# ChenWu98/cycle-diffusion

Hardware: AMD Instinct MI355X
Metric: images/sec, SD-v1.4 512px CycleDiffusion 100+100 steps, 1/2/4/8 MI355X (higher is better)
Workload: dtype fp16; 1 GPU; C2: Stable-Diffusion-v1.4-shaped U-Net + KL-f8 VAE, 512x512, custom_steps=99 white_box_steps=100 eta=0.1 skip 0, 1 trial, encoder scale 1, decoder CFG 3; batch_per_gpu=4, global_batch=4, parallelism=dp1, steps_per_launch_set=5, launch_set_cap=16, launch_sets_in_flight_per_gpu=1, images_in_flight_per_gpu=20, distributed=single process, weights=synthetic(seed=0)

## Files before the change

### cycle-diffusion_amd/csrc/attn.hip

```cpp
#include "common.h"
#include "kernels.h"

namespace cd {

namespace {

constexpr int KT = 64;

template <int DQK, int DV, int DH, int NBUF, bool VTOK, int KG, int NWV = 4>
__global__ __launch_bounds__(64 * NWV, DV <= 96 ? (KG == 32 ? (DV <= 64 ? 4 : 3) : 2) : 1) void k_attention(AttnParams p) {
  constexpr int NT = 64 * NWV;
  constexpr int KLD = DQK + 8;
  constexpr int VLD = KT + 8;
  constexpr int NKS = DQK / 16;
  constexpr int NDT = DV / 32;
  constexpr int CPR = DQK / 8;
  constexpr int NKR = (KT * CPR + NT - 1) / NT;
  constexpr bool ONES = DH > 0;
  constexpr int VS = DV <= 32 ? 32 : (DV <= 96 ? 96 : 160);
  constexpr int CPRV = ONES ? DH / 8 + 1 : DV / 8;
  constexpr int NVR = VTOK ? (KT * CPRV + NT - 1) / NT : (DV * 8 + NT - 1) / NT;
  constexpr int VBUF = VTOK ? KT * VS : DV * VLD;
  static_assert(!ONES || (DH < DV && (DH & 7) == 0 && ((DH >> 2) & 1) == 0), "ones row placement");
  __shared__ __attribute__((aligned(16))) bf16_t Ks[NBUF][KT * KLD];
  __shared__ __attribute__((aligned(16))) bf16_t Vs[NBUF][VBUF];

  const int tid = threadIdx.x, lane = tid & 63, wave = tid >> 6;
  const int qi = lane & 31, half = lane >> 5;
  const int h = blockIdx.y, b = blockIdx.z;
  const int q0 = blockIdx.x * (32 * NWV) + wave * 32;
  const int D = ONES ? DH : p.D;

  const bf16_t* qb = p.q + (int64_t)b * p.q_bs + h * D;
  const bf16_t* kb = p.k + (int64_t)b * p.k_bs + h * D;
  const bf16_t* vtb = VTOK ? p.v + (int64_t)b * p.v_bs + h * D
                           : p.vt + ((int64_t)b * p.H + h) * (int64_t)p.vt_dpad * p.vt_tpad;

  bf16x8 qf[NKS];
  const float qsc = p.scale * 1.44269504088896340736f;
  {
    const int q = q0 + qi;
#pragma unroll
    for (int ks = 0; ks < NKS; ++ks) {
      const int d0 = ks * 16 + 8 * half;
      uint4 raw = make_uint4(0, 0, 0, 0);
      if (q < p.Tq && d0 < D) raw = *(const uint4*)(qb + (int64_t)q * p.ldq + d0);
      if (!p.q_log2) {
        float f[8];
        unpack8(raw, f);
#pragma unroll
        for (int e = 0; e < 8; ++e) f[e] *= qsc;
        raw = pack8(f);
      }
      qf[ks] = *(bf16x8*)&raw;
    }
  }

  constexpr unsigned kNoLoad = 0x80000000u;
  const unsigned k_bytes = p.Tk > 0 ? (unsigned)(((int64_t)(p.Tk - 1) * p.ldk + D) * 2) : 0u;
  const unsigned v_bytes = VTOK ? (p.Tk > 0 ? (unsigned)(((int64_t)(p.Tk - 1) * p.ldv + D) * 2) : 0u)
                                : (unsigned)((int64_t)p.vt_dpad * p.vt_tpad * 2);
  const __amdgpu_buffer_rsrc_t rs_k = __builtin_amdgcn_make_buffer_rsrc((void*)kb, 0, k_bytes, 0x00020000);
  const __amdgpu_buffer_rsrc_t rs_v = __builtin_amdgcn_make_buffer_rsrc((void*)vtb, 0, v_bytes, 0x00020000);
  unsigned k_voff[NKR], v_voff[NVR];
  int k_loff[NKR], v_loff[NVR];
  bool v_ones[NVR];
#pragma unroll
  for (int i = 0; i < NKR; ++i) {
    const int id = tid + i * NT;
    const int row = id / CPR, ch = id % CPR;
    const bool ok = id < KT * CPR && ch * 8 < D;
    k_voff[i] = ok ? (unsigned)((row * p.ldk + ch * 8) * 2) : kNoLoad;
    k_loff[i] = id < KT * CPR ? row * KLD + ch * 8 : -1;
  }
#pragma unroll
  for (int i = 0; i < NVR; ++i) {
    const int id = tid + i * NT;
    if (VTOK) {
      const int row = id / CPRV, ch = id % CPRV;
      const bool data = id < KT * CPRV && ch * 8 < D;
      v_voff[i] = data ? (unsigned)((row * p.ldv + ch * 8) * 2) : kNoLoad;
      v_loff[i] = id < KT * CPRV ? row * VS + ch * 8 : -1;
      v_ones[i] = ONES && ch * 8 == DH;
    } else {
      const int row = id >> 3, ch = id & 7;
      v_voff[i] = row < DV ? (unsigned)((row * p.vt_tpad + ch * 8) * 2) : kNoLoad;
      v_loff[i] = row < DV ? row * VLD + (ch >> 1) * 16 + (ch & 1) * 4 : -1;
      v_ones[i] = ONES && row == DH;
    }
  }
  uint4 kreg[NKR], vreg[NVR];
  auto fetch = [&](int key0) {
    const unsigned k_toff = (unsigned)(key0 * p.ldk * 2);
    const unsigned v_toff = (unsigned)(VTOK ? key0 * p.ldv * 2 : key0 * 2);
#pragma unroll
    for (int i = 0; i < NKR; ++i)
      kreg[i] = __builtin_bit_cast(uint4, __builtin_amdgcn_raw_buffer_load_b128(rs_k, k_voff[i] + k_toff, 0, 0));
#pragma unroll
    for (int i = 0; i < NVR; ++i)
      vreg[i] = __builtin_bit_cast(uint4, __builtin_amdgcn_raw_buffer_load_b128(rs_v, v_voff[i] + v_toff, 0, 0));
  };
  auto commit = [&](int buf) {
#pragma unroll
    for (int i = 0; i < NKR; ++i)
      if (k_loff[i] >= 0) *(uint4*)(&Ks[buf][k_loff[i]]) = kreg[i];
#pragma unroll
    for (int i = 0; i < NVR; ++i) {
      uint4 v = vreg[i];
      if (VTOK) {
        if (v_ones[i]) v = make_uint4(kOnePair & 0xffffu, 0, 0, 0);
        if (v_loff[i] >= 0) *(uint4*)(&Vs[buf][v_loff[i]]) = v;
      } else {
        if (v_ones[i]) v = make_uint4(kOnePair, kOnePair, kOnePair, kOnePair);
        if (v_loff[i] >= 0) {
          *(uint2*)(&Vs[buf][v_loff[i]]) = make_uint2(v.x, v.y);
          *(uint2*)(&Vs[buf][v_loff[i] + 8]) = make_uint2(v.z, v.w);
        }
      }
    }
  };
  const int vtr_off = ((4 * half + ((lane & 15) >> 2)) * VS + 16 * ((lane >> 4) & 1) + 4 * (lane & 3));

  f32x16 o[NDT];
#pragma unroll
  for (int i = 0; i < NDT; ++i)
#pragma unroll
    for (int r = 0; r < 16; ++r) o[i][r] = 0.f;
  f32x16 negm;
#pragma unroll
  for (int r = 0; r < 16; ++r) negm[r] = 0.f;
  float l_part = 0.f;
  constexpr float kDefer = 8.0f;

  const int ntiles = (p.Tk + KT - 1) / KT;
  fetch(0);
  commit(0);
  __syncthreads();
  for (int t = 0; t < ntiles; ++t) {
    const int key0 = t * KT;
    const int buf = NBUF == 2 ? (t & 1) : 0;
    const bool more = t + 1 < ntiles;
    if (more) fetch(key0 + KT);
    const bf16_t* Kt = Ks[buf];
    const bf16_t* Vt = Vs[buf];

#pragma unroll
    for (int g = 0; g < KT / KG; ++g) {
      constexpr int HPG = KG / 32;
      f32x16 s[HPG];
      {
        bf16x8 kf[HPG][NKS];
#pragma unroll
        for (int kh = 0; kh < HPG; ++kh)
#pragma unroll
          for (int ks = 0; ks < NKS; ++ks)
            kf[kh][ks] = *(const bf16x8*)(Kt + ((g * HPG + kh) * 32 + qi) * KLD + ks * 16 + 8 * half);
        if (KG == 64) __builtin_amdgcn_sched_barrier(0);
#pragma unroll
        for (int ks = 0; ks < NKS; ++ks)
#pragma unroll
          for (int kh = 0; kh < HPG; ++kh)
            s[kh] = CD_MFMA_32x32x16(kf[kh][ks], qf[ks], ks == 0 ? negm : s[kh]);
      }
      if (key0 + KT > p.Tk || p.causal) {
        const int kmax = p.causal ? min(p.Tk - 1, q0 + qi) : p.Tk - 1;
#pragma unroll
        for (int kh = 0; kh < HPG; ++kh)
#pragma unroll
          for (int r = 0; r < 16; ++r) {
            const int key = key0 + (g * HPG + kh) * 32 + (r & 3) + 8 * (r >> 2) + 4 * half;
            s[kh][r] = key <= kmax ? s[kh][r] : -INFINITY;
          }
      }
      float mx = __builtin_amdgcn_fmed3f(s[HPG - 1][14], s[HPG - 1][15], INFINITY);
      if (HPG == 2) {
#pragma unroll
        for (int r = 0; r < 14; r += 2)
          asm("v_max3_f32 %0, %1, %2, %3" : "=v"(mx) : "v"(mx), "v"(s[1][r]), "v"(s[1][r + 1]));
      }
#pragma unroll
      for (int r = 0; r < (HPG == 2 ? 16 : 14); r += 2)
        asm("v_max3_f32 %0, %1, %2, %3" : "=v"(mx) : "v"(mx), "v"(s[0][r]), "v"(s[0][r + 1]));
      const bool first = t == 0 && g == 0;
      if (first || __any(mx > kDefer)) {
        const float mxq = fmaxf(mx, __shfl_xor(mx, 32));
        float delta = first ? mxq : fmaxf(mxq, 0.f);
        delta = delta == -INFINITY ? 0.f : delta;
        const float alpha = first ? 1.f : __builtin_amdgcn_exp2f(-delta);
#pragma unroll
        for (int kh = 0; kh < HPG; ++kh)
#pragma unroll
          for (int r = 0; r < 16; ++r) s[kh][r] -= delta;
#pragma unroll
        for (int r = 0; r < 16; ++r) negm[r] -= delta;
#pragma unroll
        for (int i = 0; i < NDT; ++i)
#pragma unroll
          for (int r = 0; r < 16; ++r) o[i][r] *= alpha;
        l_part *= alpha;
      }
      uint32_t pw[HPG][8];
      float ps = 0.f;
#pragma unroll
      for (int kh = 0; kh < HPG; ++kh)
#pragma unroll
        for (int r = 0; r < 16; r += 2) {
          const float e0 = __builtin_amdgcn_exp2f(s[kh][r]);
          const float e1 = __builtin_amdgcn_exp2f(s[kh][r + 1]);
          if (!ONES) ps += e0 + e1;
          pw[kh][r >> 1] = pack2_prob(e0, e1);
        }
      if (!ONES) l_part += ps;

#pragma unroll
      for (int kh = 0; kh < HPG; ++kh)
#pragma unroll
        for (int s2 = 0; s2 < 2; ++s2) {
          const uint4 praw = make_uint4(pw[kh][4 * s2], pw[kh][4 * s2 + 1], pw[kh][4 * s2 + 2], pw[kh][4 * s2 + 3]);
          const bf16x8 pf = __builtin_bit_cast(bf16x8, praw);
          const int k16 = (g * HPG + kh) * 32 + 16 * s2;
#pragma unroll
          for (int dt = 0; dt < NDT; ++dt) {
            bf16x8 vf;
            if (VTOK) {
              typedef __attribute__((address_space(3))) bf16x4* lds4_t;
              const bf16_t* vr = Vt + vtr_off + k16 * VS + dt * 32;
              const bf16x4 lo = __builtin_amdgcn_ds_read_tr16_b64_v4i16((lds4_t)vr);
              const bf16x4 hi = __builtin_amdgcn_ds_read_tr16_b64_v4i16((lds4_t)(vr + 8 * VS));
              vf = __builtin_shufflevector(lo, hi, 0, 1, 2, 3, 4, 5, 6, 7);
            } else {
              vf = *(const bf16x8*)(Vt + (dt * 32 + qi) * VLD + k16 + 8 * half);
            }
            o[dt] = CD_MFMA_32x32x16(vf, pf, o[dt]);
          }
        }
    }

    if (NBUF == 1) __syncthreads();
    if (more) commit(NBUF == 2 ? (buf ^ 1) : 0);
    __syncthreads();
  }

  float l_tot;
  if (ONES) {
    constexpr int L = DH % 32;
    const float lv = o[DH / 32][(L & 3) + 4 * (L >> 3)];
    l_tot = __shfl(lv, qi);
  } else {
    l_tot = l_part + __shfl_xor(l_part, 32);
  }
  const float inv = 1.0f / l_tot;
  const int q = q0 + qi;
  if (q < p.Tq) {
    bf16_t* ob = p.o + (int64_t)b * p.o_bs + (int64_t)q * p.ldo + h * D;
#pragma unroll
    for (int dt = 0; dt < NDT; ++dt)
#pragma unroll
      for (int rq = 0; rq < 4; ++rq) {
        const int d0 = dt * 32 + 8 * rq + 4 * half;
        if (d0 < D) {
          float bb[4] = {0.f, 0.f, 0.f, 0.f};
          if (p.obias) {
#pragma unroll
            for (int e = 0; e < 4; ++e) bb[e] = p.obias[h * D + d0 + e];
          }
          uint2 pk;
          pk.x = pack2(o[dt][rq * 4 + 0] * inv + bb[0], o[dt][rq * 4 + 1] * inv + bb[1]);
          pk.y = pack2(o[dt][rq * 4 + 2] * inv + bb[2], o[dt][rq * 4 + 3] * inv + bb[3]);
          *(uint2*)(ob + d0) = pk;
        }
      }
  }
}

template <int NWV>
__global__ __launch_bounds__(64 * NWV, 4) void k_attention_d40(AttnParams p) {
#if defined(__HIP_DEVICE_COMPILE__)
  static_assert(NWV == 8, "one K copy per wave and tile");
  typedef __attribute__((address_space(3))) void* lptr_t;
  constexpr int D = 40, NKS = 3, ROWB = 128;
  constexpr int KBUF = KT * ROWB;
  constexpr int VBUF = 48 * ROWB;
  constexpr int BUF = KBUF + VBUF;
  __shared__ __attribute__((aligned(1024))) char lds[2 * BUF];

  const int tid = threadIdx.x, lane = tid & 63;
  const int wave = __builtin_amdgcn_readfirstlane(tid >> 6);
  const int qi = lane & 31, half = lane >> 5;
  const int h = blockIdx.y, b = blockIdx.z;
  const int q0 = blockIdx.x * (32 * NWV) + wave * 32;

  const bf16_t* qb = p.q + (int64_t)b * p.q_bs + h * D;
  const bf16_t* kb = p.k + (int64_t)b * p.k_bs + h * D;
  const bf16_t* vtb = p.vt + ((int64_t)b * p.H + h) * (int64_t)p.vt_dpad * p.vt_tpad;

  bf16x8 qf[NKS];
  {
    const float qsc = p.scale * 1.44269504088896340736f;
    const int q = q0 + qi;
#pragma unroll
    for (int ks = 0; ks < NKS; ++ks) {
      const int d0 = ks * 16 + 8 * half;
      uint4 raw = make_uint4(0, 0, 0, 0);
      if (q < p.Tq && d0 < D) raw = *(const uint4*)(qb + (int64_t)q * p.ldq + d0);
      if (!p.q_log2) {
        float f[8];
        unpack8(raw, f);
#pragma unroll
        for (int e = 0; e < 8; ++e) f[e] *= qsc;
        raw = pack8(f);
      }
      qf[ks] = *(bf16x8*)&raw;
    }
  }

  constexpr unsigned kNoLoad = 0x80000000u;
  const unsigned k_bytes = p.Tk > 0 ? (unsigned)(((int64_t)(p.Tk - 1) * p.ldk + D) * 2) : 0u;
  const unsigned v_bytes = (unsigned)((int64_t)p.vt_dpad * p.vt_tpad * 2);
  const __amdgpu_buffer_rsrc_t rs_k = __builtin_amdgcn_make_buffer_rsrc((void*)kb, 0, k_bytes, 0x00020000);
  const __amdgpu_buffer_rsrc_t rs_v = __builtin_amdgcn_make_buffer_rsrc((void*)vtb, 0, v_bytes, 0x00020000);
  unsigned k_voff, v_voff;
  {
    const int row = 8 * wave + (lane >> 3);
    const int lc = (lane & 7) ^ ((row >> 1) & 7);
    const int pc = (row >> 2) & 3;
    const int key = (row & ~12) | ((((pc & 1) << 1) | (pc >> 1)) << 2);
    k_voff = lc < D / 8 ? (unsigned)((key * p.ldk + lc * 8) * 2) : kNoLoad;
    v_voff = (row < D && row < p.vt_dpad) ? (unsigned)((row * p.vt_tpad + lc * 8) * 2) : kNoLoad;
  }
  auto fetch = [&](int key0, int buf) {
    char* kd = lds + buf * BUF + wave * 1024;
    __builtin_amdgcn_raw_ptr_buffer_load_lds(rs_k, (lptr_t)kd, 16, k_voff + (unsigned)(key0 * p.ldk * 2), 0, 0, 0);
    if (wave < D / 8)
      __builtin_amdgcn_raw_ptr_buffer_load_lds(rs_v, (lptr_t)(kd + KBUF), 16, v_voff + (unsigned)(key0 * 2), 0, 0, 0);
  };
  if (wave == 5 || wave == 6) {
    const uint4 v = lane < 8 ? make_uint4(kOnePair, kOnePair, kOnePair, kOnePair) : make_uint4(0, 0, 0, 0);
    *(uint4*)(lds + (wave - 5) * BUF + KBUF + D * ROWB + lane * 16) = v;
  }

  const int sw = (qi >> 1) & 7;
  const int kf_off = qi * ROWB;
  const int vf_off = KBUF + qi * ROWB;
  const int tm = lane & 15, tg = lane >> 4;
  const int vt_off = KBUF + (32 + tm) * ROWB;
  const int vt_sw = ((32 + tm) >> 1) & 7, vt_lc = ((tg & 1) << 1) | (tg >> 1);

  f32x16 o0;
  f32x4 ot0 = {0.f, 0.f, 0.f, 0.f}, ot1 = {0.f, 0.f, 0.f, 0.f};
  f32x16 negm;
#pragma unroll
  for (int r = 0; r < 16; ++r) { o0[r] = 0.f; negm[r] = 0.f; }
  constexpr float kDefer = 8.0f;

  const int ntiles = (p.Tk + KT - 1) / KT;
  fetch(0, 0);
  asm volatile("s_waitcnt vmcnt(0)" ::: "memory");
  __syncthreads();
  for (int t = 0; t < ntiles; ++t) {
    const int key0 = t * KT;
    const int buf = t & 1;
    if (t + 1 < ntiles) fetch(key0 + KT, buf ^ 1);
    const char* Bt = lds + buf * BUF;
#pragma unroll
    for (int g = 0; g < 2; ++g) {
      f32x16 s;
      {
        bf16x8 kf[NKS];
#pragma unroll
        for (int ks = 0; ks < NKS; ++ks)
          kf[ks] = *(const bf16x8*)(Bt + kf_off + g * 32 * ROWB + (((2 * ks + half) ^ sw) << 4));
#pragma unroll
        for (int ks = 0; ks < NKS; ++ks) s = CD_MFMA_32x32x16(kf[ks], qf[ks], ks == 0 ? negm : s);
      }
      if (key0 + KT > p.Tk || p.causal) {
        const int kmax = p.causal ? min(p.Tk - 1, q0 + qi) : p.Tk - 1;
#pragma unroll
        for (int r = 0; r < 16; ++r) {
          const int row = (r & 3) + 8 * (r >> 2) + 4 * half;
          const int pc = (row >> 2) & 3;
          const int key = key0 + g * 32 + ((row & ~12) | ((((pc & 1) << 1) | (pc >> 1)) << 2));
          s[r] = key <= kmax ? s[r] : -INFINITY;
        }
      }
      float mx = __builtin_amdgcn_fmed3f(s[14], s[15], INFINITY);
#pragma unroll
      for (int r = 0; r < 14; r += 2) asm("v_max3_f32 %0, %1, %2, %3" : "=v"(mx) : "v"(mx), "v"(s[r]), "v"(s[r + 1]));
      const bool first = t == 0 && g == 0;
      if (first || __any(mx > kDefer)) {
        const float mxq = fmaxf(mx, __shfl_xor(mx, 32));
        float delta = first ? mxq : fmaxf(mxq, 0.f);
        delta = delta == -INFINITY ? 0.f : delta;
        const float alpha = first ? 1.f : __builtin_amdgcn_exp2f(-delta);
#pragma unroll
        for (int r = 0; r < 16; ++r) { s[r] -= delta; negm[r] -= delta; o0[r] *= alpha; }
        const float a0 = __shfl(alpha, lane & 15), a1 = __shfl(alpha, 16 + (lane & 15));
#pragma unroll
        for (int r = 0; r < 4; ++r) { ot0[r] *= a0; ot1[r] *= a1; }
      }
      uint32_t pw[8];
#pragma unroll
      for (int r = 0; r < 16; r += 2)
        pw[r >> 1] = pack2_prob(__builtin_amdgcn_exp2f(s[r]), __builtin_amdgcn_exp2f(s[r + 1]));
#pragma unroll
      for (int s2 = 0; s2 < 2; ++s2) {
        const bf16x8 vf = *(const bf16x8*)(Bt + vf_off + (((4 * g + 2 * s2 + half) ^ sw) << 4));
        const uint4 praw = make_uint4(pw[4 * s2], pw[4 * s2 + 1], pw[4 * s2 + 2], pw[4 * s2 + 3]);
        o0 = CD_MFMA_32x32x16(vf, __builtin_bit_cast(bf16x8, praw), o0);
      }
      {
        uint32_t xa[4], ya[4];
#pragma unroll
        for (int i = 0; i < 4; ++i) {
          const auto r2 = __builtin_amdgcn_permlane16_swap(pw[i], pw[4 + i], false, false);
          xa[i] = r2[0]; ya[i] = r2[1];
        }
        const bf16x8 va = *(const bf16x8*)(Bt + vt_off + (((4 * g + vt_lc) ^ vt_sw) << 4));
        ot0 = CD_MFMA_16x16x32(va, __builtin_bit_cast(bf16x8, make_uint4(xa[0], xa[1], xa[2], xa[3])), ot0);
        ot1 = CD_MFMA_16x16x32(va, __builtin_bit_cast(bf16x8, make_uint4(ya[0], ya[1], ya[2], ya[3])), ot1);
      }
    }
    asm volatile("s_waitcnt vmcnt(0)" ::: "memory");
    __syncthreads();
  }

  const float l0 = __shfl(ot0[0], 32 + (lane & 15)), l1 = __shfl(ot1[0], 32 + (lane & 15));
  {
    const int q = q0 + qi;
    const float inv = 1.0f / ((qi & 16) ? l1 : l0);
    if (q < p.Tq) {
      bf16_t* ob = p.o + (int64_t)b * p.o_bs + (int64_t)q * p.ldo + h * D;
#pragma unroll
      for (int rq = 0; rq < 4; ++rq) {
        const int d0 = 8 * rq + 4 * half;
        float bb[4] = {0.f, 0.f, 0.f, 0.f};
        if (p.obias) {
#pragma unroll
          for (int e = 0; e < 4; ++e) bb[e] = p.obias[h * D + d0 + e];
        }
        uint2 pk;
        pk.x = pack2(o0[rq * 4 + 0] * inv + bb[0], o0[rq * 4 + 1] * inv + bb[1]);
        pk.y = pack2(o0[rq * 4 + 2] * inv + bb[2], o0[rq * 4 + 3] * inv + bb[3]);
        *(uint2*)(ob + d0) = pk;
      }
    }
  }
  if (tg < 2) {
    const int d0 = 32 + 4 * tg;
    float bb[4] = {0.f, 0.f, 0.f, 0.f};
    if (p.obias) {
#pragma unroll
      for (int e = 0; e < 4; ++e) bb[e] = p.obias[h * D + d0 + e];
    }
#pragma unroll
    for (int qh = 0; qh < 2; ++qh) {
      const int q = q0 + tm + 16 * qh;
      const f32x4 ov = qh ? ot1 : ot0;
      const float inv = 1.0f / (qh ? l1 : l0);
      if (q < p.Tq) {
        uint2 pk;
        pk.x = pack2(ov[0] * inv + bb[0], ov[1] * inv + bb[1]);
        pk.y = pack2(ov[2] * inv + bb[2], ov[3] * inv + bb[3]);
        *(uint2*)(p.o + (int64_t)b * p.o_bs + (int64_t)q * p.ldo + h * D + d0) = pk;
      }
    }
  }
#endif
}

__global__ __launch_bounds__(256) void k_transpose_v(const bf16_t* __restrict__ v, int ldv, int64_t v_bs,
                                                     bf16_t* __restrict__ vt, int H, int Tk, int D,
                                                     int Dpad, int Tpad) {
  extern __shared__ __attribute__((aligned(16))) bf16_t tile[];
  const int key0 = blockIdx.x * 64, h = blockIdx.y, b = blockIdx.z;
  const int ldt = D + 2;
  const int cpr = D / 8;
  for (int id = threadIdx.x; id < 64 * cpr; id += 256) {
    const int row = id / cpr, ch = id % cpr;
    uint4 raw = make_uint4(0, 0, 0, 0);
    if (key0 + row < Tk) raw = *(const uint4*)(v + (int64_t)b * v_bs + (int64_t)(key0 + row) * ldv + h * D + ch * 8);
    bf16_t* d = tile + row * ldt + ch * 8;
    const bf16_t* rs = (const bf16_t*)&raw;
#pragma unroll
    for (int e = 0; e < 8; ++e) d[e] = rs[e];
  }
  __syncthreads();
  bf16_t* ob = vt + ((int64_t)b * H + h) * (int64_t)Dpad * Tpad;
  for (int id = threadIdx.x; id < Dpad * 64; id += 256) {
    const int d = id >> 6, key = id & 63;
    bf16_t val = 0;
    if (d < D) val = tile[key * ldt + d];
    ob[(int64_t)d * Tpad + key0 + key] = val;
  }
}

template <int DQK, int DV>
__global__ __launch_bounds__(256, DV <= 96 ? 2 : 1) void k_cross_attention_ctrl(CtrlAttnParams p) {
  constexpr int NT = 256, CK = kCtrlKeys, NG = CK / 32;
  constexpr int KLD = DQK + 8, NKS = DQK / 16, NDT = DV / 32, CPR = DQK / 8;
  constexpr int VS = DV <= 32 ? 32 : (DV <= 96 ? 96 : 160), CPV = VS / 8;
  __shared__ __attribute__((aligned(16))) bf16_t Ks[2][CK * KLD];
  __shared__ __attribute__((aligned(16))) bf16_t Vs[2][CK * VS];

  const int tid = threadIdx.x, lane = tid & 63, wave = tid >> 6;
  const int qi = lane & 31, half = lane >> 5;
  const int h = blockIdx.y, b = blockIdx.z, bs = b % p.B_src;
  const int q0 = blockIdx.x * 128 + wave * 32;
  const int D = p.D, L = p.L;

#pragma unroll
  for (int src = 0; src < 2; ++src) {
    const bf16_t* kb = (src == 0 ? p.k_src + (int64_t)bs * p.k_bs : p.k_own + (int64_t)b * p.k_bs) + h * D;
    const bf16_t* vb = (src == 0 ? p.va : p.vb) + (int64_t)b * p.v_bs + h * D;
    for (int id = tid; id < CK * CPR; id += NT) {
      const int row = id / CPR, ch = id % CPR;
      uint4 raw = make_uint4(0, 0, 0, 0);
      if (row < L && ch * 8 < D) raw = *(const uint4*)(kb + (int64_t)row * p.ldk + ch * 8);
      *(uint4*)(&Ks[src][row * KLD + ch * 8]) = raw;
    }
    for (int id = tid; id < CK * CPV; id += NT) {
      const int row = id / CPV, ch = id % CPV;
      uint4 raw = make_uint4(0, 0, 0, 0);
      if (row < L && ch * 8 < D) raw = *(const uint4*)(vb + (int64_t)row * p.ldv + ch * 8);
      *(uint4*)(&Vs[src][row * VS + ch * 8]) = raw;
    }
  }
  __syncthreads();

  const int vtr_off = ((4 * half + ((lane & 15) >> 2)) * VS + 16 * ((lane >> 4) & 1) + 4 * (lane & 3));
  const float qsc = p.scale * 1.44269504088896340736f;
  f32x16 o[NDT];
#pragma unroll
  for (int i = 0; i < NDT; ++i)
#pragma unroll
    for (int r = 0; r < 16; ++r) o[i][r] = 0.f;

#pragma unroll
  for (int src = 0; src < 2; ++src) {
    const bf16_t* qb = (src == 0 ? p.q_src + (int64_t)bs * p.q_bs : p.q_own + (int64_t)b * p.q_bs) + h * D;
    bf16x8 qf[NKS];
    {
      const int q = q0 + qi;
#pragma unroll
      for (int ks = 0; ks < NKS; ++ks) {
        const int d0 = ks * 16 + 8 * half;
        uint4 raw = make_uint4(0, 0, 0, 0);
        if (q < p.Tq && d0 < D) raw = *(const uint4*)(qb + (int64_t)q * p.ldq + d0);
        if (!p.q_log2) {
          float f[8];
          unpack8(raw, f);
#pragma unroll
          for (int e = 0; e < 8; ++e) f[e] *= qsc;
          raw = pack8(f);
        }
        qf[ks] = *(bf16x8*)&raw;
      }
    }
    const bf16_t* Kt = Ks[src];
    const bf16_t* Vt = Vs[src];
    f32x16 s[NG];
#pragma unroll
    for (int g = 0; g < NG; ++g) {
#pragma unroll
      for (int r = 0; r < 16; ++r) s[g][r] = 0.f;
#pragma unroll
      for (int ks = 0; ks < NKS; ++ks) {
        const bf16x8 kf = *(const bf16x8*)(Kt + (g * 32 + qi) * KLD + ks * 16 + 8 * half);
        s[g] = CD_MFMA_32x32x16(kf, qf[ks], s[g]);
      }
    }
    float mx = -INFINITY;
#pragma unroll
    for (int g = 0; g < NG; ++g)
#pragma unroll
      for (int r = 0; r < 16; ++r) {
        const int key = g * 32 + (r & 3) + 8 * (r >> 2) + 4 * half;
        s[g][r] = key < L ? s[g][r] : -INFINITY;
        mx = fmaxf(mx, s[g][r]);
      }
    mx = fmaxf(mx, __shfl_xor(mx, 32));
    float ps = 0.f;
#pragma unroll
    for (int g = 0; g < NG; ++g)
#pragma unroll
      for (int r = 0; r < 16; ++r) {
        s[g][r] = __builtin_amdgcn_exp2f(s[g][r] - mx);
        ps += s[g][r];
      }
    ps += __shfl_xor(ps, 32);
    const float inv = 256.0f / ps;
#pragma unroll
    for (int g = 0; g < NG; ++g) {
      uint32_t pw[8];
#pragma unroll
      for (int r = 0; r < 16; r += 2) pw[r >> 1] = pack2_prob(s[g][r] * inv, s[g][r + 1] * inv);
#pragma unroll
      for (int s2 = 0; s2 < 2; ++s2) {
        const uint4 praw = make_uint4(pw[4 * s2], pw[4 * s2 + 1], pw[4 * s2 + 2], pw[4 * s2 + 3]);
        const bf16x8 pf = __builtin_bit_cast(bf16x8, praw);
        const int k16 = g * 32 + 16 * s2;
#pragma unroll
        for (int dt = 0; dt < NDT; ++dt) {
          typedef __attribute__((address_space(3))) bf16x4* lds4_t;
          const bf16_t* vr = Vt + vtr_off + k16 * VS + dt * 32;
          const bf16x4 lo = __builtin_amdgcn_ds_read_tr16_b64_v4i16((lds4_t)vr);
          const bf16x4 hi = __builtin_amdgcn_ds_read_tr16_b64_v4i16((lds4_t)(vr + 8 * VS));
          const bf16x8 vf = __builtin_shufflevector(lo, hi, 0, 1, 2, 3, 4, 5, 6, 7);
          o[dt] = CD_MFMA_32x32x16(vf, pf, o[dt]);
        }
      }
    }
  }

  const int q = q0 + qi;
  if (q < p.Tq) {
    constexpr float kUnscale = 1.0f / 256.0f;
    bf16_t* ob = p.o + (int64_t)b * p.o_bs + (int64_t)q * p.ldo + h * D;
#pragma unroll
    for (int dt = 0; dt < NDT; ++dt)
#pragma unroll
      for (int rq = 0; rq < 4; ++rq) {
        const int d0 = dt * 32 + 8 * rq + 4 * half;
        if (d0 < D) {
          uint2 pk;
          pk.x = pack2(o[dt][rq * 4 + 0] * kUnscale, o[dt][rq * 4 + 1] * kUnscale);
          pk.y = pack2(o[dt][rq * 4 + 2] * kUnscale, o[dt][rq * 4 + 3] * kUnscale);
          *(uint2*)(ob + d0) = pk;
        }
      }
  }
}

__global__ __launch_bounds__(256) void k_ctrl_values(const bf16_t* __restrict__ v, const float* __restrict__ M,
                                                     const float* __restrict__ alpha, const float* __restrict__ w, int B_ctrl,
                                                     int L, int C, bf16_t* __restrict__ va, bf16_t* __restrict__ vb) {
  const int i = blockIdx.x, r = blockIdx.y, s = r % B_ctrl;
  const float* Mi = M + ((int64_t)s * L + i) * L;
  const float* al = alpha + (int64_t)s * L;
  const float* ww = w + (int64_t)s * L;
  const bf16_t* vr = v + (int64_t)r * L * C;
  const float bi = (1.0f - al[i]) * ww[i];
  for (int c = threadIdx.x; c < C; c += 256) {
    float acc = 0.f;
    for (int j = 0; j < L; ++j) {
      const float m = Mi[j] * al[j] * ww[j];
      if (m != 0.f) acc = fmaf(m, bf2f(vr[(int64_t)j * C + c]), acc);
    }
    va[((int64_t)r * L + i) * C + c] = f2bf(acc);
    vb[((int64_t)r * L + i) * C + c] = f2bf(bi * bf2f(vr[(int64_t)i * C + c]));
  }
}

}

void launch_cross_attention_ctrl(hipStream_t st, const CtrlAttnParams& p) {
  CD_CHECK(p.B > 0 && p.B_src > 0 && p.H > 0 && p.Tq > 0, "cross-attention control: empty launch");
  CD_CHECK(p.L > 0 && p.L <= kCtrlKeys, "cross-attention control: context length %d above the %d keys the kernel keeps resident",
           p.L, kCtrlKeys);
  CD_CHECK((p.ldq % 8) == 0 && (p.ldk % 8) == 0 && (p.ldv % 8) == 0 && (p.ldo % 4) == 0 && (p.q_bs % 8) == 0 &&
               (p.k_bs % 8) == 0 && (p.v_bs % 8) == 0 && (p.o_bs % 4) == 0,
           "cross-attention control: leading dims");
  CD_CHECK((((uintptr_t)p.q_own | (uintptr_t)p.q_src | (uintptr_t)p.k_own | (uintptr_t)p.k_src | (uintptr_t)p.va |
             (uintptr_t)p.vb) & 15) == 0 && ((uintptr_t)p.o & 7) == 0, "cross-attention control: pointer alignment");
  const dim3 grid(ceil_div(p.Tq, 128), p.H, p.B);
#define CD_CTRL(DQK, DV) hipLaunchKernelGGL((k_cross_attention_ctrl<DQK, DV>), grid, dim3(256), 0, st, p)
  switch (p.D) {
    case 32: CD_CTRL(32, 32); break;
    case 40: CD_CTRL(48, 64); break;
    case 64: CD_CTRL(64, 64); break;
    case 80: CD_CTRL(80, 96); break;
    case 160: CD_CTRL(160, 160); break;
    default: CD_CHECK(false, "cross-attention control: head dim %d unsupported (32, 40, 64, 80, 160)", p.D);
  }
#undef CD_CTRL
}

void launch_ctrl_values(hipStream_t st, const bf16_t* v, const float* M, const float* alpha, const float* w, int rows,
                        int B_ctrl, int L, int C, bf16_t* va, bf16_t* vb) {
  CD_CHECK(rows > 0 && B_ctrl > 0 && L > 0 && C > 0, "control values: empty launch");
  hipLaunchKernelGGL(k_ctrl_values, dim3(L, rows), dim3(256), 0, st, v, M, alpha, w, B_ctrl, L, C, va, vb);
}

void launch_attention(hipStream_t st, const AttnParams& p) {
  CD_CHECK(p.D % 8 == 0 && p.D <= 160, "attention: head dim %d unsupported by the fused kernel", p.D);
  CD_CHECK((p.v != nullptr) != (p.vt != nullptr), "attention: exactly one of v (token-major) / vt (transposed)");
  if (p.vt) CD_CHECK(p.vt_tpad % KT == 0 && p.vt_tpad >= round_up(p.Tk, KT), "attention: V^T key padding");
  else CD_CHECK((p.ldv % 8) == 0 && ((uintptr_t)p.v & 15) == 0, "attention: V row stride / alignment");
  CD_CHECK((p.ldq % 8) == 0 && (p.ldk % 8) == 0 && (p.ldo % 4) == 0, "attention: leading dims");
  dim3 grid(ceil_div(p.Tq, 128), p.H, p.B);
#define CD_LAUNCH_KG(DQK, DV, DH, NBUF, KG)                                                                  \
  do {                                                                                                      \
    if (p.v) hipLaunchKernelGGL((k_attention<DQK, DV, DH, NBUF, true, KG>), grid, dim3(256), 0, st, p);      \
    else hipLaunchKernelGGL((k_attention<DQK, DV, DH, NBUF, false, KG>), grid, dim3(256), 0, st, p);         \
  } while (0)
#define CD_ATTN(DQK, DV, DH, NBUF) CD_LAUNCH_KG(DQK, DV, DH, NBUF, 64)
  if (p.D == 40 && p.Tq >= 1024 && p.Tk >= 1024 && p.vt) {
    const bool aligned16 = ((((uintptr_t)p.q | (uintptr_t)p.k | (uintptr_t)p.vt | (uintptr_t)p.o) & 15) == 0) &&
                           (p.ldq % 8) == 0 && (p.ldk % 8) == 0 && (p.ldo % 8) == 0 && (p.q_bs % 8) == 0 && (p.k_bs % 8) == 0 &&
                           (p.o_bs % 8) == 0;
    if (p.vt_dpad >= 40 && aligned16 && (p.vt_tpad % 8) == 0 && p.vt_tpad >= ceil_div(p.Tk, 64) * 64 &&
        (int64_t)p.Tk * p.ldk * 2 < (1ll << 31) && (int64_t)p.vt_dpad * p.vt_tpad * 2 < (1ll << 31))
      hipLaunchKernelGGL((k_attention_d40<8>), dim3(ceil_div(p.Tq, 256), p.H, p.B), dim3(512), 0, st, p);
    else
      hipLaunchKernelGGL((k_attention<48, 64, 40, 2, false, 32, 8>), dim3(ceil_div(p.Tq, 256), p.H, p.B), dim3(512), 0, st,
                         p);
  } else if (p.D == 40) CD_LAUNCH_KG(48, 64, 40, 2, 32);
  else if (p.D == 80) CD_LAUNCH_KG(80, 96, 80, 2, 32);
  else if (p.D <= 32) CD_ATTN(32, 32, 0, 2);
  else if (p.D <= 48) CD_ATTN(48, 64, 0, 2);
  else if (p.D <= 64) CD_ATTN(64, 64, 0, 2);
  else if (p.D <= 80) CD_ATTN(80, 96, 0, 2);
  else if (p.D <= 96) CD_ATTN(96, 96, 0, 2);
  else if (p.D <= 128) CD_ATTN(128, 128, 0, 1);
  else CD_ATTN(160, 160, 0, 1);
#undef CD_ATTN
#undef CD_LAUNCH_KG
}

void launch_transpose_v(hipStream_t st, const bf16_t* v, int ldv, int64_t v_bs, bf16_t* vt, int B,
                        int H, int Tk, int D, int Dpad, int Tpad) {
  CD_CHECK(D % 8 == 0 && Tpad % 64 == 0, "transpose_v: D %% 8, Tpad %% 64");
  const size_t lds = (size_t)64 * (D + 2) * sizeof(bf16_t);
  hipLaunchKernelGGL(k_transpose_v, dim3(Tpad / 64, H, B), dim3(256), lds, st, v, ldv, v_bs, vt, H,
                     Tk, D, Dpad, Tpad);
}

}
```

Baseline: 3.549 images/s.

## Add slab-based cross-attention kernel keeping all short-context K/V resident in LDS

Adds a specialised cross-attention kernel for short key sequences (≤96 tokens, e.g. the 77 text tokens) with head dims 40/80/160. Each block loads a 320-channel slab of K and V for all keys into LDS once, then loops over query chunks with several heads per block, using a single-pass softmax (no online rescaling), transposed LDS reads for V, and buffer loads/stores. The grid is sized from the device CU count so work spreads across the GPU. It can be disabled with an environment variable. The trade-offs are extra specialised code, higher LDS use per block, and a fixed max-minus-8 exponent shift in the softmax.

```diff
diff --git a/cycle-diffusion_amd/csrc/attn.hip b/cycle-diffusion_amd/csrc/attn.hip
--- a/cycle-diffusion_amd/csrc/attn.hip
+++ b/cycle-diffusion_amd/csrc/attn.hip
@@ -629,6 +629,224 @@
         }
       }
   }
+}
+
+constexpr int kSlabC = 320;
+constexpr int kSlabKeys = 96;
+typedef __attribute__((ext_vector_type(2))) float f32x2;
+
+__device__ inline float prob_pair_sum(uint32_t pw, float acc) {
+#if CD_ACT_FP16
+  typedef __attribute__((ext_vector_type(2))) _Float16 h2;
+  const h2 one = {(_Float16)1.0f, (_Float16)1.0f};
+  return __builtin_amdgcn_fdot2(__builtin_bit_cast(h2, pw), one, acc, false);
+#else
+  return acc + __uint_as_float(pw << 16) + __uint_as_float(pw & 0xffff0000u);
+#endif
+}
+
+template <int D, int GR>
+__global__ __launch_bounds__(512, 1) void k_cross_attention_slab(AttnParams p, int qchunk) {
+#if defined(__HIP_DEVICE_COMPILE__)
+  constexpr int NW = 8, NT = 64 * NW, SC = kSlabC, NG = GR + 1, CK = NG * 32;
+  constexpr int HPS = SC / D;
+  constexpr int QB = 32 * NW / HPS;
+  constexpr int NKS = (D + 15) / 16, NDT = (D + 31) / 32;
+  constexpr int KROW = SC * 2;
+  constexpr int VS = SC + 32;
+  constexpr int CPR = SC / 8;
+  constexpr int NR = (CK * CPR + NT - 1) / NT;
+  static_assert(SC % D == 0 && NW % HPS == 0 && D % 8 == 0 && CK <= kSlabKeys, "slab geometry");
+  __shared__ __attribute__((aligned(1024))) char Ks[CK * KROW];
+  __shared__ __attribute__((aligned(16))) bf16_t Vs[CK * VS];
+
+  const int tid = threadIdx.x, lane = tid & 63;
+  const int wave = __builtin_amdgcn_readfirstlane(tid >> 6);
+  const int qi = lane & 31, half = lane >> 5;
+  const int slab = blockIdx.y, b = blockIdx.z;
+  const int Tk = p.Tk;
+
+  {
+    constexpr unsigned kNoLoad = 0x80000000u;
+    const bf16_t* kb = p.k + (int64_t)b * p.k_bs + slab * SC;
+    const bf16_t* vb = p.v + (int64_t)b * p.v_bs + slab * SC;
+    const unsigned k_bytes = (unsigned)(((int64_t)(Tk - 1) * p.ldk + SC) * 2);
+    const unsigned v_bytes = (unsigned)(((int64_t)(Tk - 1) * p.ldv + SC) * 2);
+    const __amdgpu_buffer_rsrc_t rs_k = __builtin_amdgcn_make_buffer_rsrc((void*)kb, 0, k_bytes, 0x00020000);
+    const __amdgpu_buffer_rsrc_t rs_v = __builtin_amdgcn_make_buffer_rsrc((void*)vb, 0, v_bytes, 0x00020000);
+    uint4 kr[NR], vr[NR];
+#pragma unroll
+    for (int i = 0; i < NR; ++i) {
+      const int id = tid + i * NT;
+      const int row = id / CPR, ch = id % CPR;
+      const bool ok = id < CK * CPR;
+      kr[i] = __builtin_bit_cast(uint4, __builtin_amdgcn_raw_buffer_load_b128(
+                                            rs_k, ok ? (unsigned)((row * p.ldk + ch * 8) * 2) : kNoLoad, 0, 0));
+      vr[i] = __builtin_bit_cast(uint4, __builtin_amdgcn_raw_buffer_load_b128(
+                                            rs_v, ok ? (unsigned)((row * p.ldv + ch * 8) * 2) : kNoLoad, 0, 0));
+    }
+#pragma unroll
+    for (int i = 0; i < NR; ++i) {
+      const int id = tid + i * NT;
+      const int row = id / CPR, ch = id % CPR;
+      if (id < CK * CPR) {
+        *(uint4*)(Ks + row * KROW + (((ch & ~7) | ((ch & 7) ^ ((row >> 1) & 7))) << 4)) = kr[i];
+        *(uint4*)(&Vs[row * VS + ch * 8]) = vr[i];
+      }
+    }
+  }
+  __syncthreads();
+
+  const int hoff = (wave % HPS) * D;
+  const int sub = wave / HPS;
+  const int qbeg = blockIdx.x * qchunk, qend = min(p.Tq, qbeg + qchunk);
+  const float qsc = p.scale * 1.44269504088896340736f;
+  constexpr unsigned kNoLane = 0x80000000u;
+  const __amdgpu_buffer_rsrc_t rs_q = __builtin_amdgcn_make_buffer_rsrc(
+      (void*)(p.q + (int64_t)b * p.q_bs + slab * SC), 0, (unsigned)(((int64_t)(p.Tq - 1) * p.ldq + SC) * 2), 0x00020000);
+  const __amdgpu_buffer_rsrc_t rs_o = __builtin_amdgcn_make_buffer_rsrc(
+      (void*)(p.o + (int64_t)b * p.o_bs + slab * SC), 0, (unsigned)(((int64_t)(p.Tq - 1) * p.ldo + SC) * 2), 0x00020000);
+
+  auto load_q = [&](int q0, uint4* raw) {
+    const int q = q0 + sub * 32 + qi;
+#pragma unroll
+    for (int ks = 0; ks < NKS; ++ks) {
+      const int d0 = ks * 16 + 8 * half;
+      const unsigned off = (q < qend && d0 < D) ? (unsigned)((q * p.ldq + hoff + d0) * 2) : kNoLane;
+      raw[ks] = __builtin_bit_cast(uint4, __builtin_amdgcn_raw_buffer_load_b128(rs_q, off, 0, 0));
+    }
+  };
+
+  const int ksw = (qi >> 1) & 7;
+  int kf_off[NKS];
+  bool kf_zero[NKS];
+#pragma unroll
+  for (int ks = 0; ks < NKS; ++ks) {
+    kf_zero[ks] = ks * 16 + 8 * half >= D;
+    const int c = hoff / 8 + 2 * ks + half - (kf_zero[ks] ? 1 : 0);
+    kf_off[ks] = qi * KROW + (((c & ~7) | ((c & 7) ^ ksw)) << 4);
+  }
+  const int vtr_off = (4 * half + ((lane & 15) >> 2)) * VS + 16 * ((lane >> 4) & 1) + 4 * (lane & 3) + hoff;
+
+  auto read_k = [&](int g, int ks) {
+    bf16x8 kf = *(const bf16x8*)(Ks + g * 32 * KROW + kf_off[ks]);
+    if (NKS * 16 > D && ks == NKS - 1 && kf_zero[ks]) kf = bf16x8{0, 0, 0, 0, 0, 0, 0, 0};
+    return kf;
+  };
+  auto read_v = [&](int g, int s2, int dt) {
+    typedef __attribute__((address_space(3))) bf16x4* lds4_t;
+    const bf16_t* vr = Vs + vtr_off + (g * 32 + 16 * s2) * VS + dt * 32;
+    const bf16x4 lo = __builtin_amdgcn_ds_read_tr16_b64_v4i16((lds4_t)vr);
+    const bf16x4 hi = __builtin_amdgcn_ds_read_tr16_b64_v4i16((lds4_t)(vr + 8 * VS));
+    return (bf16x8)__builtin_shufflevector(lo, hi, 0, 1, 2, 3, 4, 5, 6, 7);
+  };
+  f32x16 kmask, kzero;
+#pragma unroll
+  for (int r = 0; r < 16; ++r) {
+    kmask[r] = GR * 32 + (r & 3) + 8 * (r >> 2) + 4 * half < Tk ? 0.f : -INFINITY;
+    kzero[r] = 0.f;
+  }
+
+  uint4 qraw[NKS];
+  load_q(qbeg, qraw);
+  typedef decltype(__builtin_amdgcn_raw_buffer_load_b128(rs_o, 0, 0, 0)) b128_t;
+#pragma unroll
+  for (int i = 0; i < (D + 15) / 16; ++i)
+    __builtin_amdgcn_raw_buffer_store_b128(__builtin_bit_cast(b128_t, make_uint4(0, 0, 0, 0)), rs_o, kNoLane + 16u * i, 0,
+                                           0);
+  for (int q0 = qbeg; q0 < qend; q0 += QB) {
+    bf16x8 qf[NKS];
+#pragma unroll
+    for (int ks = 0; ks < NKS; ++ks) {
+      uint4 raw = qraw[ks];
+      if (!p.q_log2) {
+        float f[8];
+        unpack8(raw, f);
+#pragma unroll
+        for (int e = 0; e < 8; ++e) f[e] *= qsc;
+        raw = pack8(f);
+      }
+      qf[ks] = __builtin_bit_cast(bf16x8, raw);
+    }
+    load_q(q0 + QB, qraw);
+
+    f32x16 s[NG];
+#pragma unroll
+    for (int g = 0; g < NG; ++g) {
+      bf16x8 kf[NKS];
+#pragma unroll
+      for (int ks = 0; ks < NKS; ++ks) kf[ks] = read_k(g, ks);
+      __builtin_amdgcn_sched_barrier(0);
+#pragma unroll
+      for (int ks = 0; ks < NKS; ++ks) s[g] = CD_MFMA_32x32x16(kf[ks], qf[ks], ks == 0 ? (g == GR ? kmask : kzero) : s[g]);
+    }
+    float mg[NG];
+#pragma unroll
+    for (int g = 0; g < NG; ++g) {
+      mg[g] = __builtin_amdgcn_fmed3f(s[g][14], s[g][15], INFINITY);
+#pragma unroll
+      for (int r = 0; r < 14; r += 2)
+        asm("v_max3_f32 %0, %1, %2, %3" : "=v"(mg[g]) : "v"(mg[g]), "v"(s[g][r]), "v"(s[g][r + 1]));
+    }
+    float mx = mg[0];
+#pragma unroll
+    for (int g = 1; g < NG; ++g) mx = fmaxf(mx, mg[g]);
+    mx = fmaxf(mx, __shfl_xor(mx, 32));
+    const f32x2 mm = {mx - 8.0f, mx - 8.0f};
+    uint32_t pw[NG][8];
+    float ps = 0.f;
+#pragma unroll
+    for (int g = 0; g < NG; ++g)
+#pragma unroll
+      for (int r = 0; r < 16; r += 2) {
+        const f32x2 t = f32x2{s[g][r], s[g][r + 1]} - mm;
+        pw[g][r >> 1] = pack2_prob(__builtin_amdgcn_exp2f(t.x), __builtin_amdgcn_exp2f(t.y));
+        ps = prob_pair_sum(pw[g][r >> 1], ps);
+      }
+    ps += __shfl_xor(ps, 32);
+    const float inv1 = 1.0f / ps;
+    const f32x2 inv = {inv1, inv1};
+
+    f32x16 o[NDT];
+#pragma unroll
+    for (int i = 0; i < NDT; ++i)
+#pragma unroll
+      for (int r = 0; r < 16; ++r) o[i][r] = 0.f;
+#pragma unroll
+    for (int g = 0; g < NG; ++g)
+#pragma unroll
+      for (int s2 = 0; s2 < 2; ++s2) {
+        const uint4 praw = make_uint4(pw[g][4 * s2], pw[g][4 * s2 + 1], pw[g][4 * s2 + 2], pw[g][4 * s2 + 3]);
+        const bf16x8 pf = __builtin_bit_cast(bf16x8, praw);
+        bf16x8 vf[NDT];
+#pragma unroll
+        for (int dt = 0; dt < NDT; ++dt) vf[dt] = read_v(g, s2, dt);
+        __builtin_amdgcn_sched_barrier(0);
+#pragma unroll
+        for (int dt = 0; dt < NDT; ++dt) o[dt] = CD_MFMA_32x32x16(vf[dt], pf, o[dt]);
+      }
+
+    const int q = q0 + sub * 32 + qi;
+#pragma unroll
+    for (int dt = 0; dt < NDT; ++dt)
+#pragma unroll
+      for (int j = 0; j < 2; ++j) {
+        if (dt * 32 + 16 * j >= D) continue;
+        const int d0 = dt * 32 + 16 * j + 8 * half;
+        uint32_t w[4];
+#pragma unroll
+        for (int e = 0; e < 4; ++e) {
+          const f32x2 t = f32x2{o[dt][8 * j + 2 * e], o[dt][8 * j + 2 * e + 1]} * inv;
+          w[e] = pack2(t.x, t.y);
+        }
+        const auto lo = __builtin_amdgcn_permlane32_swap(w[0], w[2], false, false);
+        const auto hi = __builtin_amdgcn_permlane32_swap(w[1], w[3], false, false);
+        const unsigned off = (q < qend && d0 < D) ? (unsigned)((q * p.ldo + hoff + d0) * 2) : kNoLane;
+        __builtin_amdgcn_raw_buffer_store_b128(__builtin_bit_cast(b128_t, make_uint4(lo[0], hi[0], lo[1], hi[1])), rs_o, off, 0,
+                                               0);
+      }
+  }
+#endif
 }
 
 __global__ __launch_bounds__(256) void k_ctrl_values(const bf16_t* __restrict__ v, const float* __restrict__ M,
@@ -681,12 +899,70 @@
   hipLaunchKernelGGL(k_ctrl_values, dim3(L, rows), dim3(256), 0, st, v, M, alpha, w, B_ctrl, L, C, va, vb);
 }
 
+static bool cross_attn_slab_enabled() {
+  static const bool v = [] {
+    const char* e = getenv("CYCLEDIFF_CROSS_ATTN");
+    return !(e && e[0]) || atoi(e) != 0;
+  }();
+  return v;
+}
+
+static int attn_device_cus() {
+  static std::atomic<int> ncu_of[64];
+  int dev = 0;
+  HIP_CHECK(hipGetDevice(&dev));
+  int ncu = ncu_of[dev & 63].load(std::memory_order_relaxed);
+  if (!ncu) {
+    hipDeviceProp_t prop;
+    HIP_CHECK(hipGetDeviceProperties(&prop, dev));
+    ncu = prop.multiProcessorCount > 0 ? prop.multiProcessorCount : 256;
+    ncu_of[dev & 63].store(ncu, std::memory_order_relaxed);
+  }
+  return ncu;
+}
+
+static bool launch_cross_attention_slab(hipStream_t st, const AttnParams& p) {
+  if (!p.v || p.causal || p.obias || p.Tk < 1 || p.Tk > kSlabKeys) return false;
+  if (p.D != 40 && p.D != 80 && p.D != 160) return false;
+  if ((p.H * p.D) % kSlabC != 0 || p.B < 1 || p.B > 65535 || p.Tq < 1) return false;
+  if ((((uintptr_t)p.q | (uintptr_t)p.k | (uintptr_t)p.v | (uintptr_t)p.o) & 15) != 0) return false;
+  if ((p.ldq % 8) || (p.ldk % 8) || (p.ldv % 8) || (p.ldo % 8) || (p.q_bs % 8) || (p.k_bs % 8) || (p.v_bs % 8) || (p.o_bs % 8))
+    return false;
+  const int64_t lim = 1ll << 31;
+  if ((int64_t)p.Tq * p.ldq * 2 >= lim || (int64_t)p.Tq * p.ldo * 2 >= lim || (int64_t)kSlabKeys * p.ldk * 2 >= lim ||
+      (int64_t)kSlabKeys * p.ldv * 2 >= lim)
+    return false;
+  if (!cross_attn_slab_enabled()) return false;
+  const int slabs = p.H * p.D / kSlabC;
+  const int qblock = 32 * 8 / (kSlabC / p.D);
+  const int64_t per_range = (int64_t)p.B * slabs;
+  const int ranges = (int)ceil_div64((int64_t)2 * attn_device_cus(), per_range);
+  const int qr = round_up(ceil_div(p.Tq, ranges), qblock);
+  const int qchunk = qr > 256 ? qr : 256;
+  const dim3 grid(ceil_div(p.Tq, qchunk), slabs, p.B);
+#define CD_SLAB(D_, GR_) hipLaunchKernelGGL((k_cross_attention_slab<D_, GR_>), grid, dim3(512), 0, st, p, qchunk)
+#define CD_SLAB_D(D_)                 \
+  do {                                \
+    if (gr == 0) CD_SLAB(D_, 0);      \
+    else if (gr == 1) CD_SLAB(D_, 1); \
+    else CD_SLAB(D_, 2);              \
+  } while (0)
+  const int gr = (p.Tk - 1) / 32;
+  if (p.D == 40) CD_SLAB_D(40);
+  else if (p.D == 80) CD_SLAB_D(80);
+  else CD_SLAB_D(160);
+#undef CD_SLAB_D
+#undef CD_SLAB
+  return true;
+}
+
 void launch_attention(hipStream_t st, const AttnParams& p) {
   CD_CHECK(p.D % 8 == 0 && p.D <= 160, "attention: head dim %d unsupported by the fused kernel", p.D);
   CD_CHECK((p.v != nullptr) != (p.vt != nullptr), "attention: exactly one of v (token-major) / vt (transposed)");
   if (p.vt) CD_CHECK(p.vt_tpad % KT == 0 && p.vt_tpad >= round_up(p.Tk, KT), "attention: V^T key padding");
   else CD_CHECK((p.ldv % 8) == 0 && ((uintptr_t)p.v & 15) == 0, "attention: V row stride / alignment");
   CD_CHECK((p.ldq % 8) == 0 && (p.ldk % 8) == 0 && (p.ldo % 4) == 0, "attention: leading dims");
+  if (launch_cross_attention_slab(st, p)) return;
   dim3 grid(ceil_div(p.Tq, 128), p.H, p.B);
 #define CD_LAUNCH_KG(DQK, DV, DH, NBUF, KG)                                                                  \
   do {                                                                                                      \
```

After: 3.564 images/s, median of 6. No clear change (+0.4%).
